# GarciaLnk/LlamaRec

Hardware: NVIDIA B200
Metric: users_per_sec_encode_score_top20 (higher is better)
Workload: dtype bf16

## Files before the change

llamarec_b200/csrc/api_util.h:

```cpp
#pragma once

#include <cuda_runtime.h>
#include <cstdarg>
#include <cstdio>

#include "../../include/llamarec_b200.h"

namespace lrb {

char* last_error_buffer();
int set_error(int code, const char* fmt, ...);
int check_arch();
int device_sm_count();

#define LRB_CUDA_TRY(expr)                                                              \
  do {                                                                                  \
    cudaError_t _e = (expr);                                                            \
    if (_e != cudaSuccess)                                                              \
      return ::lrb::set_error(static_cast<int>(_e), "%s failed: %s", #expr,             \
                              cudaGetErrorString(_e));                                  \
  } while (0)

#define LRB_REQUIRE(cond, ...)                                                          \
  do {                                                                                  \
    if (!(cond)) return ::lrb::set_error(LRB_ERR_BAD_ARG, __VA_ARGS__);                 \
  } while (0)

inline cudaStream_t as_stream(void* s) { return reinterpret_cast<cudaStream_t>(s); }

}
```

llamarec_b200/csrc/common.cuh:

```cuda
#pragma once

#include <cuda_runtime.h>
#include <cuda_bf16.h>
#include <stdint.h>

#ifndef LRB_DEVINL
#define LRB_DEVINL __device__ __forceinline__
#endif

namespace lrb {

LRB_DEVINL int float_to_key(float f) {
  int i = __float_as_int(f);
  return i >= 0 ? i : (i ^ 0x7fffffff);
}
LRB_DEVINL float key_to_float(int k) {
  return __int_as_float(k >= 0 ? k : (k ^ 0x7fffffff));
}

LRB_DEVINL bool better(float s_a, int id_a, float s_b, int id_b) {
  return (s_a > s_b) || (s_a == s_b && id_a < id_b);
}

LRB_DEVINL uint32_t smem_u32(const void* p) {
// ... 267 lines not shown
#pragma unroll
    for (int i = 0; i < N / 3; ++i) t[i] = max3(v[3 * i], v[3 * i + 1], v[3 * i + 2]);
    if constexpr (N % 3 == 1) t[M - 1] = v[N - 1];
    if constexpr (N % 3 == 2) t[M - 1] = fmaxf(v[N - 2], v[N - 1]);
    return tree_max<M>(t);
  }
}
template <int N>
LRB_DEVINL float tree_min(const float (&v)[N]) {
  if constexpr (N == 1) return v[0];
  else if constexpr (N == 2) return fminf(v[0], v[1]);
  else if constexpr (N == 3) return min3(v[0], v[1], v[2]);
  else {
    constexpr int M = (N + 2) / 3;
    float t[M];
#pragma unroll
    for (int i = 0; i < N / 3; ++i) t[i] = min3(v[3 * i], v[3 * i + 1], v[3 * i + 2]);
    if constexpr (N % 3 == 1) t[M - 1] = v[N - 1];
    if constexpr (N % 3 == 2) t[M - 1] = fminf(v[N - 2], v[N - 1]);
    return tree_min<M>(t);
  }
}
template <int N>
LRB_DEVINL int tree_min_int(const int (&v)[N]) {
  if constexpr (N == 1) return v[0];
  else if constexpr (N == 2) return min(v[0], v[1]);
  else if constexpr (N == 3) return min(min(v[0], v[1]), v[2]);
  else {
    constexpr int M = (N + 2) / 3;
    int t[M];
#pragma unroll
    for (int i = 0; i < N / 3; ++i) t[i] = min(min(v[3 * i], v[3 * i + 1]), v[3 * i + 2]);
    if constexpr (N % 3 == 1) t[M - 1] = v[N - 1];
    if constexpr (N % 3 == 2) t[M - 1] = min(v[N - 2], v[N - 1]);
    return tree_min_int<M>(t);
  }
}
template <int N>
LRB_DEVINL int tree_sum_int(const int (&v)[N]) {
  if constexpr (N == 1) return v[0];
  else if constexpr (N == 2) return v[0] + v[1];
  else if constexpr (N == 3) return v[0] + v[1] + v[2];
  else {
    constexpr int M = (N + 2) / 3;
    int t[M];
#pragma unroll
    for (int i = 0; i < N / 3; ++i) t[i] = v[3 * i] + v[3 * i + 1] + v[3 * i + 2];
    if constexpr (N % 3 == 1) t[M - 1] = v[N - 1];
    if constexpr (N % 3 == 2) t[M - 1] = v[N - 2] + v[N - 1];
    return tree_sum_int<M>(t);
  }
}

LRB_DEVINL float4 lds_f32x4(uint32_t addr) {
  float4 v;
  asm volatile("ld.shared.v4.f32 {%0, %1, %2, %3}, [%4];"
               : "=f"(v.x), "=f"(v.y), "=f"(v.z), "=f"(v.w)
               : "r"(addr)
               : "memory");
  return v;
}
LRB_DEVINL float lds_f32(uint32_t addr) {
  float v;
  asm volatile("ld.shared.f32 %0, [%1];" : "=f"(v) : "r"(addr) : "memory");
  return v;
}
LRB_DEVINL int lds_s32(uint32_t addr) {
  int v;
  asm volatile("ld.shared.s32 %0, [%1];" : "=r"(v) : "r"(addr) : "memory");
  return v;
}
LRB_DEVINL int lds_volatile_s32(uint32_t addr) {
  int v;
  asm volatile("ld.volatile.shared.s32 %0, [%1];" : "=r"(v) : "r"(addr) : "memory");
  return v;
}
LRB_DEVINL void sts_f32(uint32_t addr, float v) {
  asm volatile("st.shared.f32 [%0], %1;" ::"r"(addr), "f"(v) : "memory");
}
LRB_DEVINL void sts_s32(uint32_t addr, int v) {
  asm volatile("st.shared.s32 [%0], %1;" ::"r"(addr), "r"(v) : "memory");
}

LRB_DEVINL long long load_id(const void* __restrict__ ids, size_t idx, int id_bytes) {
  return id_bytes == 4 ? static_cast<long long>(__ldg(static_cast<const int*>(ids) + idx))
                       : __ldg(static_cast<const long long*>(ids) + idx);
}

LRB_DEVINL float warp_sum(float v) {
#pragma unroll
  for (int o = 16; o > 0; o >>= 1) v += __shfl_xor_sync(0xffffffffu, v, o);
  return v;
}

LRB_DEVINL uint4 philox4x32_10(uint4 c, uint32_t k0, uint32_t k1) {
#pragma unroll
  for (int r = 0; r < 10; ++r) {
    if (r > 0) { k0 += 0x9E3779B9u; k1 += 0xBB67AE85u; }
    const uint32_t hi0 = __umulhi(0xD2511F53u, c.x), lo0 = 0xD2511F53u * c.x;
    const uint32_t hi1 = __umulhi(0xCD9E8D57u, c.z), lo1 = 0xCD9E8D57u * c.z;
    c = make_uint4(hi1 ^ c.y ^ k0, lo1, hi0 ^ c.w ^ k1, lo0);
  }
  return c;
}

struct DropoutSite {
  uint32_t key0, key1;
  uint32_t site;
  uint32_t thr;
  float scale;
  __host__ __device__ bool active() const { return thr != 0u; }
};

LRB_DEVINL float4 dropout_mult4(const DropoutSite& d, uint32_t t, uint32_t j4) {
  const uint4 r = philox4x32_10(make_uint4(t, j4, d.site, 0u), d.key0, d.key1);
  return make_float4(r.x >= d.thr ? d.scale : 0.f, r.y >= d.thr ? d.scale : 0.f, r.z >= d.thr ? d.scale : 0.f,
                     r.w >= d.thr ? d.scale : 0.f);
}
LRB_DEVINL float dropout_mult(const DropoutSite& d, uint32_t t, uint32_t j) {
  const float4 m = dropout_mult4(d, t, j >> 2);
  const uint32_t w = j & 3u;
  return w == 0 ? m.x : w == 1 ? m.y : w == 2 ? m.z : m.w;
}

}
```

llamarec_b200/csrc/encode.cu:

```cuda
#include "api_util.h"
#include "common.cuh"

#include <climits>

namespace lrb {
namespace enc {

constexpr int D = LRB_D;
constexpr int H2 = 2 * LRB_H;
constexpr int FF = LRB_FF;
constexpr int TOK = 64;
constexpr int THREADS = 256;
constexpr float LN_EPS = 1e-5f;

constexpr int OFF_EMB_LN_W = 0;
constexpr int OFF_EMB_LN_B = 64;
constexpr int OFF_BLOCKS = 128;
constexpr int B_LAM_RE = 0;
constexpr int B_LAM_IM = 128;
constexpr int B_GAMMA = 256;
constexpr int B_WIN_T = 384;
constexpr int B_BIN = B_WIN_T + D * H2;
constexpr int B_WOUT_T = B_BIN + H2;
constexpr int B_BOUT = B_WOUT_T + H2 * D;
constexpr int B_LN1_W = B_BOUT + D;
constexpr int B_LN1_B = B_LN1_W + D;
constexpr int B_W1_T = B_LN1_B + D;
constexpr int B_B1 = B_W1_T + D * FF;
constexpr int B_W2_T = B_B1 + FF;
constexpr int B_B2 = B_W2_T + FF * D;
constexpr int B_LN2_W = B_B2 + D;
constexpr int B_LN2_B = B_LN2_W + D;
constexpr int BLOCK_FLOATS = B_LN2_B + D;

LRB_DEVINL int user_of_token(const int* __restrict__ tok_offset, int B, int i) {
  int lo = 0, hi = B;
  while (hi - lo > 1) {
    const int mid = (lo + hi) >> 1;
    if (__ldg(tok_offset + mid) <= i) lo = mid; else hi = mid;
  }
  return lo;
}

LRB_DEVINL void gemm_k64_n256(const float* __restrict__ At, const float* __restrict__ W, int ty, int tx,
                              float (&acc)[8][8]) {
#pragma unroll
  for (int i = 0; i < 8; ++i)
#pragma unroll
    for (int j = 0; j < 8; ++j) acc[i][j] = 0.f;
#pragma unroll 4
  for (int k = 0; k < 64; ++k) {
    const float4 a0 = *reinterpret_cast<const float4*>(At + k * TOK + ty * 8);
    const float4 a1 = *reinterpret_cast<const float4*>(At + k * TOK + ty * 8 + 4);
    const float4 w0 = *reinterpret_cast<const float4*>(W + k * 256 + tx * 4);
    const float4 w1 = *reinterpret_cast<const float4*>(W + k * 256 + 128 + tx * 4);
    const float a[8] = {a0.x, a0.y, a0.z, a0.w, a1.x, a1.y, a1.z, a1.w};
    const float w[8] = {w0.x, w0.y, w0.z, w0.w, w1.x, w1.y, w1.z, w1.w};
#pragma unroll
    for (int i = 0; i < 8; ++i)
#pragma unroll
      for (int j = 0; j < 8; ++j) acc[i][j] = fmaf(a[i], w[j], acc[i][j]);
  }
}
LRB_DEVINL void gemm_k256_n64(const float* __restrict__ At, const float* __restrict__ W, int ty, int tx,
                              float (&acc)[4][4]) {
#pragma unroll
  for (int i = 0; i < 4; ++i)
#pragma unroll
    for (int j = 0; j < 4; ++j) acc[i][j] = 0.f;
#pragma unroll 8
  for (int k = 0; k < 256; ++k) {
    const float4 a4 = *reinterpret_cast<const float4*>(At + k * TOK + ty * 4);
    const float4 w4 = *reinterpret_cast<const float4*>(W + k * 64 + tx * 4);
    const float a[4] = {a4.x, a4.y, a4.z, a4.w};
    const float w[4] = {w4.x, w4.y, w4.z, w4.w};
#pragma unroll
    for (int i = 0; i < 4; ++i)
#pragma unroll
      for (int j = 0; j < 4; ++j) acc[i][j] = fmaf(a[i], w[j], acc[i][j]);
  }
}

LRB_DEVINL void copy_weights(float* dst, const float* __restrict__ src, int n_floats, int tid) {
  const float4* s4 = reinterpret_cast<const float4*>(src);
  float4* d4 = reinterpret_cast<float4*>(dst);
  for (int i = tid; i < n_floats / 4; i += THREADS) d4[i] = __ldg(s4 + i);
}

LRB_DEVINL void layernorm_rows(float* Cs, int n_rows, const float* __restrict__ w,
                               const float* __restrict__ b, float* dst_g_base,
                               const int* s_dst_row, int warp, int lane) {
  const float w0 = __ldg(w + lane), w1 = __ldg(w + lane + 32);
  const float b0 = __ldg(b + lane), b1 = __ldg(b + lane + 32);
  for (int r = warp; r < n_rows; r += THREADS / 32) {
    const float v0 = Cs[r * 65 + lane], v1 = Cs[r * 65 + lane + 32];
    const float mean = warp_sum(v0 + v1) * (1.0f / 64.0f);
    const float d0 = v0 - mean, d1 = v1 - mean;
    const float var = warp_sum(d0 * d0 + d1 * d1) * (1.0f / 64.0f);
    const float rstd = 1.0f / sqrtf(var + LN_EPS);
    const float o0 = d0 * rstd * w0 + b0;
    const float o1 = d1 * rstd * w1 + b1;
    Cs[r * 65 + lane] = o0;
    Cs[r * 65 + lane + 32] = o1;
    if (dst_g_base != nullptr) {
      const int row = s_dst_row[r];
      if (row >= 0) {
        dst_g_base[static_cast<size_t>(row) * D + lane] = o0;
        dst_g_base[static_cast<size_t>(row) * D + lane + 32] = o1;
      }
    }
  }
}

LRB_DEVINL void transpose_rows_to_kmajor(const float* Cs, float* At, int tid) {
  for (int e = tid; e < TOK * D; e += THREADS) {
    const int r = e & (TOK - 1), k = e / TOK;
    At[k * TOK + r] = Cs[r * 65 + k];
  }
}

struct InprojParams {
  const void* ids;
  int id_bytes;
  const float* table;
  long long table_rows;
  const float* wts;
  int blk;
  int first_block;
  const float* x_in;
  float* x0_out;
  float* bu;
  const int* tok_first;
  const int* tok_offset;
  int B, L;
};

constexpr int SMEM_INPROJ = (D * TOK + D * H2 + TOK * 65) * 4 + TOK * 4;

__global__ void __launch_bounds__(THREADS, 2) embed_inproj_kernel(const InprojParams p) {
  extern __shared__ __align__(16) uint8_t smem_raw[];
  float* At = reinterpret_cast<float*>(smem_raw);
  float* Ws = At + D * TOK;
  float* Cs = Ws + D * H2;
  int* s_row = reinterpret_cast<int*>(Cs + TOK * 65);
  const int tid = threadIdx.x, warp = tid >> 5, lane = tid & 31;
  const float* blkw = p.wts + OFF_BLOCKS + static_cast<size_t>(p.blk) * BLOCK_FLOATS;
  const int T = __ldg(p.tok_offset + p.B);
  const int n_tiles = (T + TOK - 1) / TOK;

  copy_weights(Ws, blkw + B_WIN_T, D * H2, tid);

  for (int tile = blockIdx.x; tile < n_tiles; tile += gridDim.x) {
    const int i0 = tile * TOK;
    __syncthreads();
    if (p.first_block) {
      for (int r = warp; r < TOK; r += THREADS / 32) {
        const int i = i0 + r;
        float v0 = 0.f, v1 = 0.f;
        if (i < T) {
          const int b = user_of_token(p.tok_offset, p.B, i);
          const int t = __ldg(p.tok_first + b) + (i - __ldg(p.tok_offset + b));
          long long id = load_id(p.ids, static_cast<size_t>(b) * p.L + t, p.id_bytes);
          if (id < 0 || id >= p.table_rows) id = 0;
          const float* row = p.table + static_cast<size_t>(id) * D;
          v0 = __ldg(row + lane);
          v1 = __ldg(row + lane + 32);
        }
        Cs[r * 65 + lane] = v0;
        Cs[r * 65 + lane + 32] = v1;
        if (lane == 0) s_row[r] = i < T ? i : -1;
      }
      __syncthreads();
      layernorm_rows(Cs, TOK, p.wts + OFF_EMB_LN_W, p.wts + OFF_EMB_LN_B, p.x0_out, s_row, warp, lane);
      __syncthreads();
      transpose_rows_to_kmajor(Cs, At, tid);
    } else {
      for (int e = tid; e < TOK * D / 4; e += THREADS) {
        const int r = e & (TOK - 1);
        const int k4 = e / TOK;
        float4 v = make_float4(0.f, 0.f, 0.f, 0.f);
        if (i0 + r < T) v = *reinterpret_cast<const float4*>(p.x_in + static_cast<size_t>(i0 + r) * D + k4 * 4);
        At[(k4 * 4 + 0) * TOK + r] = v.x;
        At[(k4 * 4 + 1) * TOK + r] = v.y;
        At[(k4 * 4 + 2) * TOK + r] = v.z;
        At[(k4 * 4 + 3) * TOK + r] = v.w;
      }
    }
    __syncthreads();

    const int ty = tid >> 5, tx = tid & 31;
    float acc[8][8];
    gemm_k64_n256(At, Ws, ty, tx, acc);
    const float4 bi0 = __ldg(reinterpret_cast<const float4*>(blkw + B_BIN + tx * 4));
    const float4 bi1 = __ldg(reinterpret_cast<const float4*>(blkw + B_BIN + 128 + tx * 4));
    const float2 g0 = __ldg(reinterpret_cast<const float2*>(blkw + B_GAMMA + tx * 2));
    const float2 g1 = __ldg(reinterpret_cast<const float2*>(blkw + B_GAMMA + 64 + tx * 2));
#pragma unroll
    for (int i = 0; i < 8; ++i) {
      const int row = i0 + ty * 8 + i;
      if (row < T) {
        float4 o0, o1;
        o0.x = (acc[i][0] + bi0.x) * g0.x; o0.y = (acc[i][1] + bi0.y) * g0.x;
        o0.z = (acc[i][2] + bi0.z) * g0.y; o0.w = (acc[i][3] + bi0.w) * g0.y;
        o1.x = (acc[i][4] + bi1.x) * g1.x; o1.y = (acc[i][5] + bi1.y) * g1.x;
        o1.z = (acc[i][6] + bi1.z) * g1.y; o1.w = (acc[i][7] + bi1.w) * g1.y;
        float* dst = p.bu + static_cast<size_t>(row) * H2;
        *reinterpret_cast<float4*>(dst + tx * 4) = o0;
        *reinterpret_cast<float4*>(dst + 128 + tx * 4) = o1;
      }
    }
  }
}

struct ScanParams {
  float2* bu;
  const void* ids;
  int id_bytes;
  const float* wts;
  int blk;
  const int* tok_first;
  const int* tok_offset;
  int B, L, levels;
  int last_only;
  float2* h_last;
};

constexpr int MAX_LEVELS = 8;
constexpr int SCAN_CHUNK = 8;

__global__ void __launch_bounds__(128) lru_scan_kernel(const ScanParams p) {
  __shared__ unsigned char s_mask[LRB_MAX_LEN];
  const int b = blockIdx.x;
  const int c = threadIdx.x;
  const int first = __ldg(p.tok_first + b);
  const int base = __ldg(p.tok_offset + b);
  const int n = __ldg(p.tok_offset + b + 1) - base;
  const int off = (1 << p.levels) - p.L;
  for (int t = c; t < p.L; t += 128) s_mask[t] = load_id(p.ids, static_cast<size_t>(b) * p.L + t, p.id_bytes) > 0 ? 1 : 0;
  __syncthreads();
  const float* blkw = p.wts + OFF_BLOCKS + static_cast<size_t>(p.blk) * BLOCK_FLOATS;
  const float lr = __ldg(blkw + B_LAM_RE + c), li = __ldg(blkw + B_LAM_IM + c);
  float qr[MAX_LEVELS], qi[MAX_LEVELS];
#pragma unroll
  for (int l = 0; l < MAX_LEVELS; ++l) { qr[l] = 0.f; qi[l] = 0.f; }

  float2* row = p.bu + static_cast<size_t>(base) * LRB_H + c;

  bool monotone = true;
  for (int t = first + 1 + c; t < p.L; t += 128) monotone = monotone && !(s_mask[t - 1] != 0 && s_mask[t] == 0);
  if (__syncthreads_and(monotone ? 1 : 0)) {
    float hr = 0.f, hi = 0.f;
    for (int j0 = 0; j0 < n; j0 += SCAN_CHUNK) {
      float2 v[SCAN_CHUNK];
#pragma unroll
      for (int u = 0; u < SCAN_CHUNK; ++u)
        v[u] = (j0 + u < n) ? row[static_cast<size_t>(j0 + u) * LRB_H] : make_float2(0.f, 0.f);
#pragma unroll
      for (int u = 0; u < SCAN_CHUNK; ++u) {
        const int j = j0 + u;
        if (j < n) {
          const float nr = v[u].x + (hr * lr - hi * li);
          const float ni = v[u].y + (hr * li + hi * lr);
          if (!p.last_only) row[static_cast<size_t>(j) * LRB_H] = make_float2(nr, ni);
          else if (j == n - 1) p.h_last[static_cast<size_t>(b) * LRB_H + c] = make_float2(nr, ni);
          const bool m = s_mask[first + j] != 0;
          hr = m ? nr : 0.f;
          hi = m ? ni : 0.f;
        }
      }
    }
    return;
  }

  for (int j0 = 0; j0 < n; j0 += SCAN_CHUNK) {
    float2 v[SCAN_CHUNK];
#pragma unroll
    for (int u = 0; u < SCAN_CHUNK; ++u)
      v[u] = (j0 + u < n) ? row[static_cast<size_t>(j0 + u) * LRB_H] : make_float2(0.f, 0.f);
#pragma unroll
    for (int u = 0; u < SCAN_CHUNK; ++u) {
      const int j = j0 + u;
      if (j < n) {
        const int t = first + j;
        const int pos = t + off;
        float ar = v[u].x, ai = v[u].y;
        float sr = 0.f, si = 0.f;
        int zlev = -1;
        bool below_all_ones = true;
#pragma unroll
        for (int l = 0; l < MAX_LEVELS; ++l) {
          if (l < p.levels) {
            const bool bit = (pos >> l) & 1;
            if (bit) {
              ar += qr[l];
              ai += qi[l];
            } else if (below_all_ones) {
              sr = ar; si = ai; zlev = l;
              below_all_ones = false;
            }
          }
        }
        if (!p.last_only) row[static_cast<size_t>(j) * LRB_H] = make_float2(ar, ai);
        else if (j == n - 1) p.h_last[static_cast<size_t>(b) * LRB_H + c] = make_float2(ar, ai);
        const float m = s_mask[t] ? 1.f : 0.f;
#pragma unroll
        for (int l = 0; l < MAX_LEVELS; ++l) {
          if (l < p.levels) {
            float xr = qr[l], xi = qi[l];
            if (l == zlev) { xr = sr * m; xi = si * m; }
            qr[l] = xr * lr - xi * li;
            qi[l] = xr * li + xi * lr;
          }
        }
      }
    }
  }
}

struct OutParams {
  const float* h;
  const float* x_res;
  const float* wts;
  int blk;
  float* x_out;
  __nv_bfloat16* out_bf16;
  const int* tok_offset;
  int B;
  int last_only;
};

constexpr int SMEM_OUT = (H2 * TOK + H2 * D + D * TOK + TOK * 65 + TOK * 65) * 4 + TOK * 4;

__global__ void __launch_bounds__(THREADS, 1) outproj_ffn_kernel(const OutParams p) {
  extern __shared__ __align__(16) uint8_t smem_raw[];
  float* Ht = reinterpret_cast<float*>(smem_raw);
  float* Ws = Ht + H2 * TOK;
  float* Yt = Ws + H2 * D;
  float* Cs = Yt + D * TOK;
  float* Ys = Cs + TOK * 65;
  int* s_row = reinterpret_cast<int*>(Ys + TOK * 65);
  const int tid = threadIdx.x, warp = tid >> 5, lane = tid & 31;
  const float* blkw = p.wts + OFF_BLOCKS + static_cast<size_t>(p.blk) * BLOCK_FLOATS;
  const int T = __ldg(p.tok_offset + p.B);
  const int n_rows_total = p.last_only ? p.B : T;
  const int n_tiles = (n_rows_total + TOK - 1) / TOK;

  for (int tile = blockIdx.x; tile < n_tiles; tile += gridDim.x) {
    const int i0 = tile * TOK;
    __syncthreads();
    for (int e = tid; e < TOK * H2 / 4; e += THREADS) {
      const int r = e & (TOK - 1);
      const int k4 = e / TOK;
      float4 v = make_float4(0.f, 0.f, 0.f, 0.f);
      if (i0 + r < n_rows_total) v = *reinterpret_cast<const float4*>(p.h + static_cast<size_t>(i0 + r) * H2 + k4 * 4);
      Ht[(k4 * 4 + 0) * TOK + r] = v.x;
      Ht[(k4 * 4 + 1) * TOK + r] = v.y;
      Ht[(k4 * 4 + 2) * TOK + r] = v.z;
      Ht[(k4 * 4 + 3) * TOK + r] = v.w;
    }
    for (int e = tid; e < TOK * D; e += THREADS) {
      const int r = e >> 6, k = e & 63;
      float v = 0.f;
      const int i = i0 + r;
      if (i < n_rows_total) {
        const int src = p.last_only ? (__ldg(p.tok_offset + i + 1) - 1) : i;
        v = p.x_res[static_cast<size_t>(src) * D + k];
      }
      Cs[r * 65 + k] = v;
    }
    if (tid < TOK) s_row[tid] = (i0 + tid < n_rows_total) ? i0 + tid : -1;
    copy_weights(Ws, blkw + B_WOUT_T, H2 * D, tid);
    __syncthreads();

    const int ty = tid >> 4, tx = tid & 15;
    {
      float acc[4][4];
      gemm_k256_n64(Ht, Ws, ty, tx, acc);
      const float4 bo = __ldg(reinterpret_cast<const float4*>(blkw + B_BOUT + tx * 4));
#pragma unroll
      for (int i = 0; i < 4; ++i) {
        const int r = ty * 4 + i;
        Cs[r * 65 + tx * 4 + 0] += acc[i][0] + bo.x;
        Cs[r * 65 + tx * 4 + 1] += acc[i][1] + bo.y;
        Cs[r * 65 + tx * 4 + 2] += acc[i][2] + bo.z;
        Cs[r * 65 + tx * 4 + 3] += acc[i][3] + bo.w;
      }
    }
    __syncthreads();
    layernorm_rows(Cs, TOK, blkw + B_LN1_W, blkw + B_LN1_B, nullptr, s_row, warp, lane);
    copy_weights(Ws, blkw + B_W1_T, D * FF, tid);
    __syncthreads();
    for (int e = tid; e < TOK * D; e += THREADS) {
      const int r = e & (TOK - 1), k = e / TOK;
      const float yv = Cs[r * 65 + k];
      Yt[k * TOK + r] = yv;
      Ys[r * 65 + k] = yv;
    }
    __syncthreads();
    {
      const int ty8 = tid >> 5, tx8 = tid & 31;
      float acc[8][8];
      gemm_k64_n256(Yt, Ws, ty8, tx8, acc);
      const float4 b0 = __ldg(reinterpret_cast<const float4*>(blkw + B_B1 + tx8 * 4));
      const float4 b1 = __ldg(reinterpret_cast<const float4*>(blkw + B_B1 + 128 + tx8 * 4));
      const float bb[8] = {b0.x, b0.y, b0.z, b0.w, b1.x, b1.y, b1.z, b1.w};
      __syncthreads();
#pragma unroll
      for (int j = 0; j < 8; ++j) {
        const int col = (j < 4 ? tx8 * 4 + j : 128 + tx8 * 4 + (j - 4));
        float4 o0, o1;
        float v[8];
#pragma unroll
        for (int i = 0; i < 8; ++i) {
          const float z = acc[i][j] + bb[j];
          v[i] = 0.5f * z * (1.0f + erff(z * 0.70710678118654752440f));
        }
        o0 = make_float4(v[0], v[1], v[2], v[3]);
        o1 = make_float4(v[4], v[5], v[6], v[7]);
        *reinterpret_cast<float4*>(Ht + col * TOK + ty8 * 8) = o0;
        *reinterpret_cast<float4*>(Ht + col * TOK + ty8 * 8 + 4) = o1;
      }
    }
    __syncthreads();
    copy_weights(Ws, blkw + B_W2_T, FF * D, tid);
    __syncthreads();
    {
      float acc[4][4];
      gemm_k256_n64(Ht, Ws, ty, tx, acc);
      const float4 b2 = __ldg(reinterpret_cast<const float4*>(blkw + B_B2 + tx * 4));
#pragma unroll
      for (int i = 0; i < 4; ++i) {
        const int r = ty * 4 + i;
        Cs[r * 65 + tx * 4 + 0] = acc[i][0] + b2.x + Ys[r * 65 + tx * 4 + 0];
        Cs[r * 65 + tx * 4 + 1] = acc[i][1] + b2.y + Ys[r * 65 + tx * 4 + 1];
        Cs[r * 65 + tx * 4 + 2] = acc[i][2] + b2.z + Ys[r * 65 + tx * 4 + 2];
        Cs[r * 65 + tx * 4 + 3] = acc[i][3] + b2.w + Ys[r * 65 + tx * 4 + 3];
      }
    }
    __syncthreads();
    layernorm_rows(Cs, TOK, blkw + B_LN2_W, blkw + B_LN2_B, p.x_out, s_row, warp, lane);
    if (p.out_bf16 != nullptr) {
      for (int r = warp; r < TOK; r += THREADS / 32) {
        const int rowi = s_row[r];
        if (rowi < 0) continue;
        p.out_bf16[static_cast<size_t>(rowi) * D + lane] = __float2bfloat16_rn(Cs[r * 65 + lane]);
        p.out_bf16[static_cast<size_t>(rowi) * D + lane + 32] = __float2bfloat16_rn(Cs[r * 65 + lane + 32]);
      }
    }
  }
}

inline size_t align256(size_t x) { return (x + 255) & ~static_cast<size_t>(255); }

}
}

extern "C" {

size_t lrb_encoder_weight_floats(int n_blocks) {
  return static_cast<size_t>(lrb::enc::OFF_BLOCKS) + static_cast<size_t>(n_blocks) * lrb::enc::BLOCK_FLOATS;
}

size_t lrb_encode_workspace_bytes(int B, int L, int all_positions) {
  using namespace lrb::enc;
  (void)all_positions;
  const size_t T = static_cast<size_t>(B) * L;
  return 2 * align256(T * D * 4) + align256(T * H2 * 4) + align256(static_cast<size_t>(B) * H2 * 4);
}

int lrb_encode_fwd(const void* ids, int id_bytes, int B, int L, const float* table_f32, int64_t table_rows,
                   const float* weights, int n_blocks, int all_positions, const int32_t* tok_first,
                   const int32_t* tok_offset, float* out_f32, void* out_bf16, void* workspace,
                   size_t workspace_bytes, void* stream) {
  using namespace lrb;
  using namespace lrb::enc;
  int rc = check_arch();
  if (rc != LRB_OK) return rc;
  LRB_REQUIRE(ids && table_f32 && weights && tok_first && tok_offset && out_f32 && workspace,
              "lrb_encode_fwd: null pointer");
  LRB_REQUIRE(B > 0 && L > 0 && n_blocks >= 1 && table_rows > 0, "lrb_encode_fwd: bad shape");
  LRB_REQUIRE(id_bytes == 4 || id_bytes == 8, "lrb_encode_fwd: id_bytes must be 4 (int32) or 8 (int64)");
  if (L > LRB_MAX_LEN)
    return set_error(LRB_ERR_UNSUPPORTED, "sequence length %d exceeds LRB_MAX_LEN=%d", L, LRB_MAX_LEN);
  if (workspace_bytes < lrb_encode_workspace_bytes(B, L, all_positions))
    return set_error(LRB_ERR_WORKSPACE, "lrb_encode_fwd: workspace too small");
  LRB_REQUIRE(!(all_positions && out_bf16 != nullptr), "lrb_encode_fwd: out_bf16 is an eval-mode output");
  cudaStream_t st = as_stream(stream);
  const size_t T = static_cast<size_t>(B) * L;
  uint8_t* ws = static_cast<uint8_t*>(workspace);
  float* xa = reinterpret_cast<float*>(ws);
  float* xb = reinterpret_cast<float*>(ws + align256(T * D * 4));
  float* bu = reinterpret_cast<float*>(ws + 2 * align256(T * D * 4));
  float* h_last = reinterpret_cast<float*>(ws + 2 * align256(T * D * 4) + align256(T * H2 * 4));
  int levels = 0;
  while ((1 << levels) < L) ++levels;

  LRB_CUDA_TRY(cudaFuncSetAttribute(embed_inproj_kernel, cudaFuncAttributeMaxDynamicSharedMemorySize, SMEM_INPROJ));
  LRB_CUDA_TRY(cudaFuncSetAttribute(outproj_ffn_kernel, cudaFuncAttributeMaxDynamicSharedMemorySize, SMEM_OUT));
  const int sms = device_sm_count();
  const int max_tiles = static_cast<int>((T + TOK - 1) / TOK);
  const int grid_tok = max_tiles < 2 * sms ? max_tiles : 2 * sms;

  float* x_cur = xa;
  float* x_nxt = xb;
  for (int blk = 0; blk < n_blocks; ++blk) {
    const bool last_blk = blk == n_blocks - 1;
    const bool last_only = last_blk && !all_positions;
    InprojParams ip;
    ip.ids = ids; ip.id_bytes = id_bytes;
    ip.table = table_f32; ip.table_rows = table_rows; ip.wts = weights; ip.blk = blk;
    ip.first_block = blk == 0 ? 1 : 0;
    ip.x_in = x_cur; ip.x0_out = blk == 0 ? x_cur : nullptr; ip.bu = bu;
    ip.tok_first = tok_first; ip.tok_offset = tok_offset; ip.B = B; ip.L = L;
    embed_inproj_kernel<<<grid_tok, THREADS, SMEM_INPROJ, st>>>(ip);
    LRB_CUDA_TRY(cudaGetLastError());

    ScanParams sp;
    sp.bu = reinterpret_cast<float2*>(bu);
    sp.ids = ids; sp.id_bytes = id_bytes;
    sp.wts = weights; sp.blk = blk; sp.tok_first = tok_first; sp.tok_offset = tok_offset;
    sp.B = B; sp.L = L; sp.levels = levels; sp.last_only = last_only ? 1 : 0;
    sp.h_last = reinterpret_cast<float2*>(h_last);
    lru_scan_kernel<<<B, 128, 0, st>>>(sp);
    LRB_CUDA_TRY(cudaGetLastError());

    OutParams op;
    op.h = last_only ? h_last : bu;
    op.x_res = x_cur; op.wts = weights; op.blk = blk;
    op.x_out = last_blk ? out_f32 : x_nxt;
    op.out_bf16 = last_only ? static_cast<__nv_bfloat16*>(out_bf16) : nullptr;
    op.tok_offset = tok_offset; op.B = B; op.last_only = last_only ? 1 : 0;
    const int tiles = last_only ? (B + TOK - 1) / TOK : max_tiles;
    const int grid = tiles < sms ? tiles : sms;
    outproj_ffn_kernel<<<grid, THREADS, SMEM_OUT, st>>>(op);
    LRB_CUDA_TRY(cudaGetLastError());
    float* tmp = x_cur; x_cur = x_nxt; x_nxt = tmp;
  }
  return LRB_OK;
}

}
```

llamarec_b200/csrc/prep.cu:

```cuda
#include "api_util.h"
#include "common.cuh"

#include <climits>

namespace lrb {
namespace {

__global__ void prepare_table_kernel(const float* __restrict__ table, const float* __restrict__ bias,
                                     long long row_begin, long long rows, __nv_bfloat16* __restrict__ out,
                                     float* __restrict__ bias_pad, uint4* __restrict__ bias_blk,
                                     long long rows_pad) {
  const long long n4 = rows * (LRB_D / 4);
  const long long stride = static_cast<long long>(gridDim.x) * blockDim.x;
  const float4* src = reinterpret_cast<const float4*>(table + row_begin * LRB_D);
  for (long long i = static_cast<long long>(blockIdx.x) * blockDim.x + threadIdx.x; i < n4; i += stride) {
    const float4 v = src[i];
    __nv_bfloat162 lo = __floats2bfloat162_rn(v.x, v.y);
    __nv_bfloat162 hi = __floats2bfloat162_rn(v.z, v.w);
    uint2 pk;
    pk.x = *reinterpret_cast<uint32_t*>(&lo);
    pk.y = *reinterpret_cast<uint32_t*>(&hi);
    reinterpret_cast<uint2*>(out)[i] = pk;
  }
  for (long long i = static_cast<long long>(blockIdx.x) * blockDim.x + threadIdx.x; i < rows_pad; i += stride) {
    const float bv = i < rows ? bias[row_begin + i] : -INFINITY;
    bias_pad[i] = bv;
    if (bias_blk != nullptr) {
      const __nv_bfloat16 hi = __float2bfloat16_rn(bv);
      float rest = i < rows ? bv - __bfloat162float(hi) : 0.f;
      const __nv_bfloat16 mid = __float2bfloat16_rn(rest);
      rest = i < rows ? rest - __bfloat162float(mid) : 0.f;
      const __nv_bfloat16 lo = __float2bfloat16_rn(rest);
      uint4 k_lo;
      k_lo.x = static_cast<uint32_t>(__bfloat16_as_ushort(hi)) |
               (static_cast<uint32_t>(__bfloat16_as_ushort(mid)) << 16);
      k_lo.y = static_cast<uint32_t>(__bfloat16_as_ushort(lo));
      k_lo.z = 0u; k_lo.w = 0u;
      bias_blk[2 * i] = k_lo;
      bias_blk[2 * i + 1] = make_uint4(0u, 0u, 0u, 0u);
    }
  }
}

constexpr int SEQ_THREADS = 128;

__global__ void __launch_bounds__(SEQ_THREADS)
prepare_sequences_kernel(const void* __restrict__ ids, int id_bytes, int B, int L, int all_positions,
                         int* __restrict__ tok_first, int* __restrict__ tok_offset,
                         int* __restrict__ excl_sorted, uint32_t* __restrict__ excl_bloom, int stride) {
  __shared__ int s_ids[LRB_MAX_LEN + 1];
  __shared__ int s_first;
  __shared__ uint32_t s_bloom[4];
  const int b = blockIdx.x;
  const int tid = threadIdx.x;
  if (tid == 0) s_first = L;
  if (tid < 4) s_bloom[tid] = 0u;
  __syncthreads();
  for (int t = tid; t < L; t += SEQ_THREADS) {
    const int id = static_cast<int>(load_id(ids, static_cast<size_t>(b) * L + t, id_bytes));
    s_ids[t] = id;
    if (id > 0) atomicMin(&s_first, t);
  }
  if (tid == 0) s_ids[L] = 0;
  __syncthreads();
  if (tid == 0) {
    int first = all_positions ? 0 : s_first;
    if (first >= L) first = L - 1;
    tok_first[b] = first;
    tok_offset[b + 1] = L - first;
    if (b == 0) tok_offset[0] = 0;
  }
  if (excl_sorted == nullptr) return;
  const int n = L + 1;
  int* out = excl_sorted + static_cast<size_t>(b) * stride;
  for (int t = tid; t < n; t += SEQ_THREADS) {
    const int v = s_ids[t];
    int rank = 0;
    for (int j = 0; j < n; ++j) {
      const int w = s_ids[j];
      rank += (w < v) || (w == v && j < t);
    }
    out[rank] = v;
    atomicOr(&s_bloom[(v >> 5) & 3], 1u << (v & 31));
  }
  for (int t = n + tid; t < stride; t += SEQ_THREADS) out[t] = INT_MAX;
  __syncthreads();
  if (tid < 4) excl_bloom[static_cast<size_t>(b) * 4 + tid] = s_bloom[tid];
}

__global__ void __launch_bounds__(1024) scan_counts_kernel(int* __restrict__ tok_offset, int B) {
  __shared__ int s_warp[32];
  __shared__ int s_carry;
  const int tid = threadIdx.x;
  const int lane = tid & 31, warp = tid >> 5;
  if (tid == 0) s_carry = 0;
  __syncthreads();
  for (int base = 0; base < B; base += 1024) {
    const int i = base + tid;
    int v = i < B ? tok_offset[i + 1] : 0;
#pragma unroll
    for (int o = 1; o < 32; o <<= 1) {
      int n = __shfl_up_sync(0xffffffffu, v, o);
      if (lane >= o) v += n;
    }
    if (lane == 31) s_warp[warp] = v;
    __syncthreads();
    if (warp == 0) {
      int w = s_warp[lane];
#pragma unroll
      for (int o = 1; o < 32; o <<= 1) {
        int n = __shfl_up_sync(0xffffffffu, w, o);
        if (lane >= o) w += n;
      }
      s_warp[lane] = w;
    }
    __syncthreads();
    const int prefix = s_carry + (warp > 0 ? s_warp[warp - 1] : 0);
    if (i < B) tok_offset[i + 1] = prefix + v;
    __syncthreads();
    if (tid == 1023) s_carry = prefix + v;
    __syncthreads();
  }
}

}
}

extern "C" {

int lrb_excl_stride(int L) { return ((L + 1) + 3) & ~3; }

size_t lrb_bias_blk_bytes(int64_t rows) { return static_cast<size_t>((rows + 255) / 256) * 8192; }

int lrb_prepare_table(const float* table_f32, const float* bias_f32, int64_t row_begin, int64_t rows,
                      void* table_bf16, float* bias_pad, void* bias_blk, void* stream) {
  using namespace lrb;
  LRB_REQUIRE(table_f32 && bias_f32 && table_bf16 && bias_pad, "lrb_prepare_table: null pointer");
  LRB_REQUIRE(rows > 0 && row_begin >= 0, "lrb_prepare_table: bad row range");
  int rc = check_arch();
  if (rc != LRB_OK) return rc;
  const long long rows_pad = (rows + 255) / 256 * 256;
  int sms = device_sm_count();
  prepare_table_kernel<<<sms * 8, 256, 0, as_stream(stream)>>>(
      table_f32, bias_f32, row_begin, rows, static_cast<__nv_bfloat16*>(table_bf16), bias_pad,
      static_cast<uint4*>(bias_blk), rows_pad);
  LRB_CUDA_TRY(cudaGetLastError());
  return LRB_OK;
}

int lrb_prepare_sequences(const void* ids, int id_bytes, int B, int L, int all_positions, int32_t* tok_first,
                          int32_t* tok_offset, int32_t* excl_sorted, uint32_t* excl_bloom, void* stream) {
  using namespace lrb;
  LRB_REQUIRE(ids && tok_first && tok_offset, "lrb_prepare_sequences: null pointer");
  LRB_REQUIRE(B > 0 && L > 0, "lrb_prepare_sequences: bad shape");
  LRB_REQUIRE(id_bytes == 4 || id_bytes == 8, "lrb_prepare_sequences: id_bytes must be 4 (int32) or 8 (int64)");
  if (L > LRB_MAX_LEN)
    return set_error(LRB_ERR_UNSUPPORTED, "sequence length %d exceeds LRB_MAX_LEN=%d", L, LRB_MAX_LEN);
  LRB_REQUIRE((excl_sorted == nullptr) == (excl_bloom == nullptr), "lrb_prepare_sequences: exclusion list and bloom filter must come together");
  int rc = check_arch();
  if (rc != LRB_OK) return rc;
  cudaStream_t st = as_stream(stream);
  prepare_sequences_kernel<<<B, SEQ_THREADS, 0, st>>>(ids, id_bytes, B, L, all_positions, tok_first, tok_offset, excl_sorted,
                                                       excl_bloom, lrb_excl_stride(L));
  LRB_CUDA_TRY(cudaGetLastError());
  scan_counts_kernel<<<1, 1024, 0, st>>>(tok_offset, B);
  LRB_CUDA_TRY(cudaGetLastError());
  return LRB_OK;
}

}
```

Baseline: 833,500.

## Pipeline outproj/FFN with cp.async double buffering, variable tiles, and PDL launches

Rewrites the output-projection/FFN kernel to stream activations and weights in 64-wide K chunks through double-buffered cp.async shared-memory slots. It uses row-major padded activations and a templated tile size (128 or 16 rows) chosen by token count, with grid size taken from an occupancy query. All encode and prep kernels are launched with programmatic dependent launch so prologues such as weight copies overlap the previous kernel's tail. The embedding gather is split so ids are resolved once per row before the loads. Risks include PDL ordering hazards and extra shared-memory and register pressure from the larger tile variant.

Result: no change. 838,500 (median of 6 runs) (+0.6%).

```diff
diff --git a/llamarec_b200/csrc/api_util.h b/llamarec_b200/csrc/api_util.h
--- a/llamarec_b200/csrc/api_util.h
+++ b/llamarec_b200/csrc/api_util.h
@@ -28,4 +28,20 @@
 
 inline cudaStream_t as_stream(void* s) { return reinterpret_cast<cudaStream_t>(s); }
 
+template <typename... Params, typename... Args>
+cudaError_t launch_kernel(void (*kernel)(Params...), unsigned grid, unsigned block, size_t smem, cudaStream_t st,
+                          bool pdl, Args... args) {
+  cudaLaunchConfig_t cfg = {};
+  cfg.gridDim = dim3(grid);
+  cfg.blockDim = dim3(block);
+  cfg.dynamicSmemBytes = smem;
+  cfg.stream = st;
+  cudaLaunchAttribute attr[1];
+  attr[0].id = cudaLaunchAttributeProgrammaticStreamSerialization;
+  attr[0].val.programmaticStreamSerializationAllowed = 1;
+  cfg.attrs = attr;
+  cfg.numAttrs = pdl ? 1 : 0;
+  return cudaLaunchKernelEx(&cfg, kernel, args...);
 }
+
+}
diff --git a/llamarec_b200/csrc/common.cuh b/llamarec_b200/csrc/common.cuh
--- a/llamarec_b200/csrc/common.cuh
+++ b/llamarec_b200/csrc/common.cuh
@@ -373,6 +373,14 @@
   asm volatile("st.shared.s32 [%0], %1;" ::"r"(addr), "r"(v) : "memory");
 }
 
+LRB_DEVINL void cp_async16(void* smem_dst, const void* gsrc) {
+  asm volatile("cp.async.cg.shared.global [%0], [%1], 16;" ::"r"(smem_u32(smem_dst)), "l"(gsrc) : "memory");
+}
+LRB_DEVINL void cp_async_wait_all() { asm volatile("cp.async.wait_all;" ::: "memory"); }
+
+LRB_DEVINL void pdl_wait() { asm volatile("griddepcontrol.wait;" ::: "memory"); }
+LRB_DEVINL void pdl_launch_dependents() { asm volatile("griddepcontrol.launch_dependents;" ::: "memory"); }
+
 LRB_DEVINL long long load_id(const void* __restrict__ ids, size_t idx, int id_bytes) {
   return id_bytes == 4 ? static_cast<long long>(__ldg(static_cast<const int*>(ids) + idx))
                        : __ldg(static_cast<const long long*>(ids) + idx);
diff --git a/llamarec_b200/csrc/encode.cu b/llamarec_b200/csrc/encode.cu
--- a/llamarec_b200/csrc/encode.cu
+++ b/llamarec_b200/csrc/encode.cu
@@ -62,46 +62,28 @@
       for (int j = 0; j < 8; ++j) acc[i][j] = fmaf(a[i], w[j], acc[i][j]);
   }
 }
-LRB_DEVINL void gemm_k256_n64(const float* __restrict__ At, const float* __restrict__ W, int ty, int tx,
-                              float (&acc)[4][4]) {
-#pragma unroll
-  for (int i = 0; i < 4; ++i)
-#pragma unroll
-    for (int j = 0; j < 4; ++j) acc[i][j] = 0.f;
-#pragma unroll 8
-  for (int k = 0; k < 256; ++k) {
-    const float4 a4 = *reinterpret_cast<const float4*>(At + k * TOK + ty * 4);
-    const float4 w4 = *reinterpret_cast<const float4*>(W + k * 64 + tx * 4);
-    const float a[4] = {a4.x, a4.y, a4.z, a4.w};
-    const float w[4] = {w4.x, w4.y, w4.z, w4.w};
-#pragma unroll
-    for (int i = 0; i < 4; ++i)
-#pragma unroll
-      for (int j = 0; j < 4; ++j) acc[i][j] = fmaf(a[i], w[j], acc[i][j]);
-  }
-}
-
 LRB_DEVINL void copy_weights(float* dst, const float* __restrict__ src, int n_floats, int tid) {
   const float4* s4 = reinterpret_cast<const float4*>(src);
   float4* d4 = reinterpret_cast<float4*>(dst);
   for (int i = tid; i < n_floats / 4; i += THREADS) d4[i] = __ldg(s4 + i);
 }
 
+template <int LD>
 LRB_DEVINL void layernorm_rows(float* Cs, int n_rows, const float* __restrict__ w,
                                const float* __restrict__ b, float* dst_g_base,
                                const int* s_dst_row, int warp, int lane) {
   const float w0 = __ldg(w + lane), w1 = __ldg(w + lane + 32);
   const float b0 = __ldg(b + lane), b1 = __ldg(b + lane + 32);
   for (int r = warp; r < n_rows; r += THREADS / 32) {
-    const float v0 = Cs[r * 65 + lane], v1 = Cs[r * 65 + lane + 32];
+    const float v0 = Cs[r * LD + lane], v1 = Cs[r * LD + lane + 32];
     const float mean = warp_sum(v0 + v1) * (1.0f / 64.0f);
     const float d0 = v0 - mean, d1 = v1 - mean;
     const float var = warp_sum(d0 * d0 + d1 * d1) * (1.0f / 64.0f);
     const float rstd = 1.0f / sqrtf(var + LN_EPS);
     const float o0 = d0 * rstd * w0 + b0;
     const float o1 = d1 * rstd * w1 + b1;
-    Cs[r * 65 + lane] = o0;
-    Cs[r * 65 + lane + 32] = o1;
+    Cs[r * LD + lane] = o0;
+    Cs[r * LD + lane + 32] = o1;
     if (dst_g_base != nullptr) {
       const int row = s_dst_row[r];
       if (row >= 0) {
@@ -135,43 +117,55 @@
   int B, L;
 };
 
-constexpr int SMEM_INPROJ = (D * TOK + D * H2 + TOK * 65) * 4 + TOK * 4;
+constexpr int SMEM_INPROJ = (D * TOK + D * H2 + TOK * 65) * 4 + TOK * 4 + TOK * 8;
 
 __global__ void __launch_bounds__(THREADS, 2) embed_inproj_kernel(const InprojParams p) {
   extern __shared__ __align__(16) uint8_t smem_raw[];
   float* At = reinterpret_cast<float*>(smem_raw);
   float* Ws = At + D * TOK;
   float* Cs = Ws + D * H2;
-  int* s_row = reinterpret_cast<int*>(Cs + TOK * 65);
+  long long* s_src = reinterpret_cast<long long*>(Cs + TOK * 65);
+  int* s_row = reinterpret_cast<int*>(s_src + TOK);
   const int tid = threadIdx.x, warp = tid >> 5, lane = tid & 31;
   const float* blkw = p.wts + OFF_BLOCKS + static_cast<size_t>(p.blk) * BLOCK_FLOATS;
+
+  copy_weights(Ws, blkw + B_WIN_T, D * H2, tid);
+  pdl_wait();
   const int T = __ldg(p.tok_offset + p.B);
   const int n_tiles = (T + TOK - 1) / TOK;
-
-  copy_weights(Ws, blkw + B_WIN_T, D * H2, tid);
 
   for (int tile = blockIdx.x; tile < n_tiles; tile += gridDim.x) {
     const int i0 = tile * TOK;
     __syncthreads();
     if (p.first_block) {
-      for (int r = warp; r < TOK; r += THREADS / 32) {
-        const int i = i0 + r;
-        float v0 = 0.f, v1 = 0.f;
+      if (tid < TOK) {
+        const int i = i0 + tid;
+        long long id = -1;
         if (i < T) {
           const int b = user_of_token(p.tok_offset, p.B, i);
           const int t = __ldg(p.tok_first + b) + (i - __ldg(p.tok_offset + b));
-          long long id = load_id(p.ids, static_cast<size_t>(b) * p.L + t, p.id_bytes);
+          id = load_id(p.ids, static_cast<size_t>(b) * p.L + t, p.id_bytes);
           if (id < 0 || id >= p.table_rows) id = 0;
+        }
+        s_src[tid] = id;
+        s_row[tid] = i < T ? i : -1;
+      }
+      __syncthreads();
+#pragma unroll
+      for (int rr = 0; rr < TOK / (THREADS / 32); ++rr) {
+        const int r = warp + rr * (THREADS / 32);
+        const long long id = s_src[r];
+        float v0 = 0.f, v1 = 0.f;
+        if (id >= 0) {
           const float* row = p.table + static_cast<size_t>(id) * D;
           v0 = __ldg(row + lane);
           v1 = __ldg(row + lane + 32);
         }
         Cs[r * 65 + lane] = v0;
         Cs[r * 65 + lane + 32] = v1;
-        if (lane == 0) s_row[r] = i < T ? i : -1;
       }
       __syncthreads();
-      layernorm_rows(Cs, TOK, p.wts + OFF_EMB_LN_W, p.wts + OFF_EMB_LN_B, p.x0_out, s_row, warp, lane);
+      layernorm_rows<65>(Cs, TOK, p.wts + OFF_EMB_LN_W, p.wts + OFF_EMB_LN_B, p.x0_out, s_row, warp, lane);
       __syncthreads();
       transpose_rows_to_kmajor(Cs, At, tid);
     } else {
@@ -210,6 +204,7 @@
       }
     }
   }
+  pdl_launch_dependents();
 }
 
 struct ScanParams {
@@ -237,6 +232,7 @@
   const int n = __ldg(p.tok_offset + b + 1) - base;
   const int off = (1 << p.levels) - p.L;
   for (int t = c; t < p.L; t += 128) s_mask[t] = load_id(p.ids, static_cast<size_t>(b) * p.L + t, p.id_bytes) > 0 ? 1 : 0;
+  pdl_wait();
   __syncthreads();
   const float* blkw = p.wts + OFF_BLOCKS + static_cast<size_t>(p.blk) * BLOCK_FLOATS;
   const float lr = __ldg(blkw + B_LAM_RE + c), li = __ldg(blkw + B_LAM_IM + c);
@@ -269,6 +265,7 @@
         }
       }
     }
+    pdl_launch_dependents();
     return;
   }
 
@@ -315,6 +312,7 @@
       }
     }
   }
+  pdl_launch_dependents();
 }
 
 struct OutParams {
@@ -329,126 +327,179 @@
   int last_only;
 };
 
-constexpr int SMEM_OUT = (H2 * TOK + H2 * D + D * TOK + TOK * 65 + TOK * 65) * 4 + TOK * 4;
-
+constexpr int LDA = 68;
+constexpr int WCH = 64 * 64;
+
+template <int TOKR>
+struct OutSmem {
+  static constexpr int ACT = TOKR * LDA;
+  static constexpr int SLOT = ACT + WCH > 2 * WCH ? ACT + WCH : 2 * WCH;
+  static constexpr int BYTES = (2 * SLOT + 2 * ACT) * 4 + TOKR * 4;
+};
+
+template <int RM>
+LRB_DEVINL void gemm_rows_k64(const float* __restrict__ A, const float* __restrict__ W, int ty, int tx,
+                              float (&acc)[RM][4]) {
+#pragma unroll 2
+  for (int k0 = 0; k0 < 64; k0 += 4) {
+    float4 a[RM], w[4];
+#pragma unroll
+    for (int i = 0; i < RM; ++i) a[i] = *reinterpret_cast<const float4*>(A + (ty + 16 * i) * LDA + k0);
+#pragma unroll
+    for (int kk = 0; kk < 4; ++kk) w[kk] = *reinterpret_cast<const float4*>(W + (k0 + kk) * 64 + tx * 4);
+#pragma unroll
+    for (int kk = 0; kk < 4; ++kk) {
+#pragma unroll
+      for (int i = 0; i < RM; ++i) {
+        const float av = kk == 0 ? a[i].x : kk == 1 ? a[i].y : kk == 2 ? a[i].z : a[i].w;
+        acc[i][0] = fmaf(av, w[kk].x, acc[i][0]);
+        acc[i][1] = fmaf(av, w[kk].y, acc[i][1]);
+        acc[i][2] = fmaf(av, w[kk].z, acc[i][2]);
+        acc[i][3] = fmaf(av, w[kk].w, acc[i][3]);
+      }
+    }
+  }
+}
+
+template <int TOKR>
+LRB_DEVINL void out_stage_load(const OutParams& p, const float* blkw, int n_rows, int i0, int s, float* slot,
+                               float* Cs, int tid) {
+  if (s < 4) {
+    for (int e = tid; e < TOKR * 16; e += THREADS) {
+      const int r = e >> 4, q = e & 15;
+      const int i = min(i0 + r, n_rows - 1);
+      cp_async16(slot + r * LDA + q * 4, p.h + static_cast<size_t>(i) * H2 + s * 64 + q * 4);
+    }
+    const float* w = blkw + B_WOUT_T + s * 64 * D;
+    for (int e = tid; e < WCH / 4; e += THREADS) cp_async16(slot + OutSmem<TOKR>::ACT + e * 4, w + e * 4);
+    if (s == 1) {
+      for (int e = tid; e < TOKR * 16; e += THREADS) {
+        const int r = e >> 4, q = e & 15;
+        const int i = min(i0 + r, n_rows - 1);
+        const int src = p.last_only ? (__ldg(p.tok_offset + i + 1) - 1) : i;
+        cp_async16(Cs + r * LDA + q * 4, p.x_res + static_cast<size_t>(src) * D + q * 4);
+      }
+    }
+  } else {
+    const int c = s - 4;
+    for (int e = tid; e < WCH / 4; e += THREADS) {
+      const int k = e >> 4, q = e & 15;
+      cp_async16(slot + k * 64 + q * 4, blkw + B_W1_T + k * FF + c * 64 + q * 4);
+    }
+    const float* w2 = blkw + B_W2_T + c * 64 * D;
+    for (int e = tid; e < WCH / 4; e += THREADS) cp_async16(slot + WCH + e * 4, w2 + e * 4);
+  }
+}
+
+template <int TOKR>
 __global__ void __launch_bounds__(THREADS, 1) outproj_ffn_kernel(const OutParams p) {
+  constexpr int RM = TOKR / 16;
+  using S = OutSmem<TOKR>;
   extern __shared__ __align__(16) uint8_t smem_raw[];
-  float* Ht = reinterpret_cast<float*>(smem_raw);
-  float* Ws = Ht + H2 * TOK;
-  float* Yt = Ws + H2 * D;
-  float* Cs = Yt + D * TOK;
-  float* Ys = Cs + TOK * 65;
-  int* s_row = reinterpret_cast<int*>(Ys + TOK * 65);
+  float* slots = reinterpret_cast<float*>(smem_raw);
+  float* Cs = slots + 2 * S::SLOT;
+  float* Fs = Cs + S::ACT;
+  int* s_row = reinterpret_cast<int*>(Fs + S::ACT);
   const int tid = threadIdx.x, warp = tid >> 5, lane = tid & 31;
+  const int ty = tid >> 4, tx = tid & 15;
   const float* blkw = p.wts + OFF_BLOCKS + static_cast<size_t>(p.blk) * BLOCK_FLOATS;
-  const int T = __ldg(p.tok_offset + p.B);
-  const int n_rows_total = p.last_only ? p.B : T;
-  const int n_tiles = (n_rows_total + TOK - 1) / TOK;
+
+  pdl_wait();
+  const int n_rows = p.last_only ? p.B : __ldg(p.tok_offset + p.B);
+  const int n_tiles = (n_rows + TOKR - 1) / TOKR;
+  if (static_cast<int>(blockIdx.x) < n_tiles)
+    out_stage_load<TOKR>(p, blkw, n_rows, blockIdx.x * TOKR, 0, slots, Cs, tid);
 
   for (int tile = blockIdx.x; tile < n_tiles; tile += gridDim.x) {
-    const int i0 = tile * TOK;
+    const int i0 = tile * TOKR;
+    const int next_tile = tile + gridDim.x;
+    auto begin_stage = [&](int s) {
+      cp_async_wait_all();
+      __syncthreads();
+      if (s < 7) out_stage_load<TOKR>(p, blkw, n_rows, i0, s + 1, slots + ((s + 1) & 1) * S::SLOT, Cs, tid);
+      else if (next_tile < n_tiles) out_stage_load<TOKR>(p, blkw, n_rows, next_tile * TOKR, 0, slots, Cs, tid);
+      return slots + (s & 1) * S::SLOT;
+    };
+
+    float acc[RM][4];
+#pragma unroll
+    for (int i = 0; i < RM; ++i)
+#pragma unroll
+      for (int j = 0; j < 4; ++j) acc[i][j] = 0.f;
+
+    for (int s = 0; s < 4; ++s) {
+      const float* slot = begin_stage(s);
+      if (s == 0 && tid < TOKR) s_row[tid] = (i0 + tid < n_rows) ? i0 + tid : -1;
+      gemm_rows_k64<RM>(slot, slot + S::ACT, ty, tx, acc);
+    }
+    {
+      const float4 bo = __ldg(reinterpret_cast<const float4*>(blkw + B_BOUT + tx * 4));
+#pragma unroll
+      for (int i = 0; i < RM; ++i) {
+        float* c = Cs + (ty + 16 * i) * LDA + tx * 4;
+        c[0] += acc[i][0] + bo.x;
+        c[1] += acc[i][1] + bo.y;
+        c[2] += acc[i][2] + bo.z;
+        c[3] += acc[i][3] + bo.w;
+      }
+    }
     __syncthreads();
-    for (int e = tid; e < TOK * H2 / 4; e += THREADS) {
-      const int r = e & (TOK - 1);
-      const int k4 = e / TOK;
-      float4 v = make_float4(0.f, 0.f, 0.f, 0.f);
-      if (i0 + r < n_rows_total) v = *reinterpret_cast<const float4*>(p.h + static_cast<size_t>(i0 + r) * H2 + k4 * 4);
-      Ht[(k4 * 4 + 0) * TOK + r] = v.x;
-      Ht[(k4 * 4 + 1) * TOK + r] = v.y;
-      Ht[(k4 * 4 + 2) * TOK + r] = v.z;
-      Ht[(k4 * 4 + 3) * TOK + r] = v.w;
-    }
-    for (int e = tid; e < TOK * D; e += THREADS) {
-      const int r = e >> 6, k = e & 63;
-      float v = 0.f;
-      const int i = i0 + r;
-      if (i < n_rows_total) {
-        const int src = p.last_only ? (__ldg(p.tok_offset + i + 1) - 1) : i;
-        v = p.x_res[static_cast<size_t>(src) * D + k];
-      }
-      Cs[r * 65 + k] = v;
-    }
-    if (tid < TOK) s_row[tid] = (i0 + tid < n_rows_total) ? i0 + tid : -1;
-    copy_weights(Ws, blkw + B_WOUT_T, H2 * D, tid);
+    layernorm_rows<LDA>(Cs, TOKR, blkw + B_LN1_W, blkw + B_LN1_B, nullptr, s_row, warp, lane);
+
+#pragma unroll
+    for (int i = 0; i < RM; ++i)
+#pragma unroll
+      for (int j = 0; j < 4; ++j) acc[i][j] = 0.f;
+    for (int c = 0; c < 4; ++c) {
+      const float* slot = begin_stage(4 + c);
+      float f[RM][4];
+#pragma unroll
+      for (int i = 0; i < RM; ++i)
+#pragma unroll
+        for (int j = 0; j < 4; ++j) f[i][j] = 0.f;
+      gemm_rows_k64<RM>(Cs, slot, ty, tx, f);
+      const float4 b1 = __ldg(reinterpret_cast<const float4*>(blkw + B_B1 + c * 64 + tx * 4));
+      const float bb[4] = {b1.x, b1.y, b1.z, b1.w};
+#pragma unroll
+      for (int i = 0; i < RM; ++i) {
+        float v[4];
+#pragma unroll
+        for (int j = 0; j < 4; ++j) {
+          const float z = f[i][j] + bb[j];
+          v[j] = 0.5f * z * (1.0f + erff(z * 0.70710678118654752440f));
+        }
+        *reinterpret_cast<float4*>(Fs + (ty + 16 * i) * LDA + tx * 4) = make_float4(v[0], v[1], v[2], v[3]);
+      }
+      __syncthreads();
+      gemm_rows_k64<RM>(Fs, slot + WCH, ty, tx, acc);
+    }
+    {
+      const float4 b2 = __ldg(reinterpret_cast<const float4*>(blkw + B_B2 + tx * 4));
+#pragma unroll
+      for (int i = 0; i < RM; ++i) {
+        float* c = Cs + (ty + 16 * i) * LDA + tx * 4;
+        c[0] = acc[i][0] + b2.x + c[0];
+        c[1] = acc[i][1] + b2.y + c[1];
+        c[2] = acc[i][2] + b2.z + c[2];
+        c[3] = acc[i][3] + b2.w + c[3];
+      }
+    }
     __syncthreads();
-
-    const int ty = tid >> 4, tx = tid & 15;
-    {
-      float acc[4][4];
-      gemm_k256_n64(Ht, Ws, ty, tx, acc);
-      const float4 bo = __ldg(reinterpret_cast<const float4*>(blkw + B_BOUT + tx * 4));
-#pragma unroll
-      for (int i = 0; i < 4; ++i) {
-        const int r = ty * 4 + i;
-        Cs[r * 65 + tx * 4 + 0] += acc[i][0] + bo.x;
-        Cs[r * 65 + tx * 4 + 1] += acc[i][1] + bo.y;
-        Cs[r * 65 + tx * 4 + 2] += acc[i][2] + bo.z;
-        Cs[r * 65 + tx * 4 + 3] += acc[i][3] + bo.w;
-      }
-    }
-    __syncthreads();
-    layernorm_rows(Cs, TOK, blkw + B_LN1_W, blkw + B_LN1_B, nullptr, s_row, warp, lane);
-    copy_weights(Ws, blkw + B_W1_T, D * FF, tid);
-    __syncthreads();
-    for (int e = tid; e < TOK * D; e += THREADS) {
-      const int r = e & (TOK - 1), k = e / TOK;
-      const float yv = Cs[r * 65 + k];
-      Yt[k * TOK + r] = yv;
-      Ys[r * 65 + k] = yv;
-    }
-    __syncthreads();
-    {
-      const int ty8 = tid >> 5, tx8 = tid & 31;
-      float acc[8][8];
-      gemm_k64_n256(Yt, Ws, ty8, tx8, acc);
-      const float4 b0 = __ldg(reinterpret_cast<const float4*>(blkw + B_B1 + tx8 * 4));
-      const float4 b1 = __ldg(reinterpret_cast<const float4*>(blkw + B_B1 + 128 + tx8 * 4));
-      const float bb[8] = {b0.x, b0.y, b0.z, b0.w, b1.x, b1.y, b1.z, b1.w};
-      __syncthreads();
-#pragma unroll
-      for (int j = 0; j < 8; ++j) {
-        const int col = (j < 4 ? tx8 * 4 + j : 128 + tx8 * 4 + (j - 4));
-        float4 o0, o1;
-        float v[8];
-#pragma unroll
-        for (int i = 0; i < 8; ++i) {
-          const float z = acc[i][j] + bb[j];
-          v[i] = 0.5f * z * (1.0f + erff(z * 0.70710678118654752440f));
-        }
-        o0 = make_float4(v[0], v[1], v[2], v[3]);
-        o1 = make_float4(v[4], v[5], v[6], v[7]);
-        *reinterpret_cast<float4*>(Ht + col * TOK + ty8 * 8) = o0;
-        *reinterpret_cast<float4*>(Ht + col * TOK + ty8 * 8 + 4) = o1;
-      }
-    }
-    __syncthreads();
-    copy_weights(Ws, blkw + B_W2_T, FF * D, tid);
-    __syncthreads();
-    {
-      float acc[4][4];
-      gemm_k256_n64(Ht, Ws, ty, tx, acc);
-      const float4 b2 = __ldg(reinterpret_cast<const float4*>(blkw + B_B2 + tx * 4));
-#pragma unroll
-      for (int i = 0; i < 4; ++i) {
-        const int r = ty * 4 + i;
-        Cs[r * 65 + tx * 4 + 0] = acc[i][0] + b2.x + Ys[r * 65 + tx * 4 + 0];
-        Cs[r * 65 + tx * 4 + 1] = acc[i][1] + b2.y + Ys[r * 65 + tx * 4 + 1];
-        Cs[r * 65 + tx * 4 + 2] = acc[i][2] + b2.z + Ys[r * 65 + tx * 4 + 2];
-        Cs[r * 65 + tx * 4 + 3] = acc[i][3] + b2.w + Ys[r * 65 + tx * 4 + 3];
-      }
-    }
-    __syncthreads();
-    layernorm_rows(Cs, TOK, blkw + B_LN2_W, blkw + B_LN2_B, p.x_out, s_row, warp, lane);
+    layernorm_rows<LDA>(Cs, TOKR, blkw + B_LN2_W, blkw + B_LN2_B, p.x_out, s_row, warp, lane);
     if (p.out_bf16 != nullptr) {
-      for (int r = warp; r < TOK; r += THREADS / 32) {
+      for (int r = warp; r < TOKR; r += THREADS / 32) {
         const int rowi = s_row[r];
         if (rowi < 0) continue;
-        p.out_bf16[static_cast<size_t>(rowi) * D + lane] = __float2bfloat16_rn(Cs[r * 65 + lane]);
-        p.out_bf16[static_cast<size_t>(rowi) * D + lane + 32] = __float2bfloat16_rn(Cs[r * 65 + lane + 32]);
-      }
-    }
-  }
-}
+        p.out_bf16[static_cast<size_t>(rowi) * D + lane] = __float2bfloat16_rn(Cs[r * LDA + lane]);
+        p.out_bf16[static_cast<size_t>(rowi) * D + lane + 32] = __float2bfloat16_rn(Cs[r * LDA + lane + 32]);
+      }
+    }
+  }
+  pdl_launch_dependents();
+}
+
+constexpr int OUT_TILE_BIG = 128;
+constexpr int OUT_TILE_SMALL = 16;
 
 inline size_t align256(size_t x) { return (x + 255) & ~static_cast<size_t>(255); }
 
@@ -495,11 +546,18 @@
   int levels = 0;
   while ((1 << levels) < L) ++levels;
 
-  LRB_CUDA_TRY(cudaFuncSetAttribute(embed_inproj_kernel, cudaFuncAttributeMaxDynamicSharedMemorySize, SMEM_INPROJ));
-  LRB_CUDA_TRY(cudaFuncSetAttribute(outproj_ffn_kernel, cudaFuncAttributeMaxDynamicSharedMemorySize, SMEM_OUT));
   const int sms = device_sm_count();
   const int max_tiles = static_cast<int>((T + TOK - 1) / TOK);
   const int grid_tok = max_tiles < 2 * sms ? max_tiles : 2 * sms;
+  LRB_CUDA_TRY(cudaFuncSetAttribute(embed_inproj_kernel, cudaFuncAttributeMaxDynamicSharedMemorySize, SMEM_INPROJ));
+  const bool big_tiles = (T + OUT_TILE_BIG - 1) / OUT_TILE_BIG >= static_cast<size_t>(sms);
+  void (*out_kernel_all)(OutParams) =
+      big_tiles ? outproj_ffn_kernel<OUT_TILE_BIG> : outproj_ffn_kernel<OUT_TILE_SMALL>;
+  const int out_tile_all = big_tiles ? OUT_TILE_BIG : OUT_TILE_SMALL;
+  for (int k = 0; k < 2; ++k)
+    LRB_CUDA_TRY(cudaFuncSetAttribute(k ? outproj_ffn_kernel<OUT_TILE_BIG> : outproj_ffn_kernel<OUT_TILE_SMALL>,
+                                      cudaFuncAttributeMaxDynamicSharedMemorySize,
+                                      k ? OutSmem<OUT_TILE_BIG>::BYTES : OutSmem<OUT_TILE_SMALL>::BYTES));
 
   float* x_cur = xa;
   float* x_nxt = xb;
@@ -512,8 +570,7 @@
     ip.first_block = blk == 0 ? 1 : 0;
     ip.x_in = x_cur; ip.x0_out = blk == 0 ? x_cur : nullptr; ip.bu = bu;
     ip.tok_first = tok_first; ip.tok_offset = tok_offset; ip.B = B; ip.L = L;
-    embed_inproj_kernel<<<grid_tok, THREADS, SMEM_INPROJ, st>>>(ip);
-    LRB_CUDA_TRY(cudaGetLastError());
+    LRB_CUDA_TRY(launch_kernel(embed_inproj_kernel, grid_tok, THREADS, SMEM_INPROJ, st, blk > 0, ip));
 
     ScanParams sp;
     sp.bu = reinterpret_cast<float2*>(bu);
@@ -521,8 +578,7 @@
     sp.wts = weights; sp.blk = blk; sp.tok_first = tok_first; sp.tok_offset = tok_offset;
     sp.B = B; sp.L = L; sp.levels = levels; sp.last_only = last_only ? 1 : 0;
     sp.h_last = reinterpret_cast<float2*>(h_last);
-    lru_scan_kernel<<<B, 128, 0, st>>>(sp);
-    LRB_CUDA_TRY(cudaGetLastError());
+    LRB_CUDA_TRY(launch_kernel(lru_scan_kernel, B, 128, 0, st, true, sp));
 
     OutParams op;
     op.h = last_only ? h_last : bu;
@@ -530,10 +586,15 @@
     op.x_out = last_blk ? out_f32 : x_nxt;
     op.out_bf16 = last_only ? static_cast<__nv_bfloat16*>(out_bf16) : nullptr;
     op.tok_offset = tok_offset; op.B = B; op.last_only = last_only ? 1 : 0;
-    const int tiles = last_only ? (B + TOK - 1) / TOK : max_tiles;
-    const int grid = tiles < sms ? tiles : sms;
-    outproj_ffn_kernel<<<grid, THREADS, SMEM_OUT, st>>>(op);
-    LRB_CUDA_TRY(cudaGetLastError());
+    void (*out_kernel)(OutParams) = last_only ? outproj_ffn_kernel<OUT_TILE_SMALL> : out_kernel_all;
+    const int out_tile = last_only ? OUT_TILE_SMALL : out_tile_all;
+    const int out_smem = out_tile == OUT_TILE_BIG ? OutSmem<OUT_TILE_BIG>::BYTES : OutSmem<OUT_TILE_SMALL>::BYTES;
+    int per_sm = 0;
+    LRB_CUDA_TRY(cudaOccupancyMaxActiveBlocksPerMultiprocessor(&per_sm, out_kernel, THREADS, out_smem));
+    const long long tiles = last_only ? (B + out_tile - 1) / out_tile : static_cast<long long>((T + out_tile - 1) / out_tile);
+    const long long resident = static_cast<long long>(per_sm > 0 ? per_sm : 1) * sms;
+    LRB_CUDA_TRY(launch_kernel(out_kernel, static_cast<unsigned>(tiles < resident ? tiles : resident), THREADS,
+                               out_smem, st, true, op));
     float* tmp = x_cur; x_cur = x_nxt; x_nxt = tmp;
   }
   return LRB_OK;
diff --git a/llamarec_b200/csrc/prep.cu b/llamarec_b200/csrc/prep.cu
--- a/llamarec_b200/csrc/prep.cu
+++ b/llamarec_b200/csrc/prep.cu
@@ -63,6 +63,7 @@
   }
   if (tid == 0) s_ids[L] = 0;
   __syncthreads();
+  pdl_launch_dependents();
   if (tid == 0) {
     int first = all_positions ? 0 : s_first;
     if (first >= L) first = L - 1;
@@ -94,6 +95,7 @@
   const int tid = threadIdx.x;
   const int lane = tid & 31, warp = tid >> 5;
   if (tid == 0) s_carry = 0;
+  pdl_wait();
   __syncthreads();
   for (int base = 0; base < B; base += 1024) {
     const int i = base + tid;
@@ -163,8 +165,7 @@
   prepare_sequences_kernel<<<B, SEQ_THREADS, 0, st>>>(ids, id_bytes, B, L, all_positions, tok_first, tok_offset, excl_sorted,
                                                        excl_bloom, lrb_excl_stride(L));
   LRB_CUDA_TRY(cudaGetLastError());
-  scan_counts_kernel<<<1, 1024, 0, st>>>(tok_offset, B);
-  LRB_CUDA_TRY(cudaGetLastError());
+  LRB_CUDA_TRY(launch_kernel(scan_counts_kernel, 1, 1024, 0, st, true, tok_offset, B));
   return LRB_OK;
 }
 
```
